# transferia/transferia

Hardware: NVIDIA H100
Metric: ChangeItems/sec on ClickBench-shaped 99-col batches (filter_rows + cast + ClickHouse native block + LZ4 frames) (higher is better)
Workload: dtype u8

## Files before the change

### transferia_b200/csrc/kernels_encode.cuh

```cuda
#pragma once
#include "device_types.cuh"

namespace tfk {

__device__ __forceinline__ uint32_t warp_incl_scan(uint32_t v) {
    const unsigned lane = threadIdx.x & 31;
#pragma unroll
    for (int d = 1; d < 32; d <<= 1) { uint32_t t = __shfl_up_sync(0xffffffffu, v, d); if (lane >= (unsigned)d) v += t; }
    return v;
}
__device__ __forceinline__ uint32_t block_excl_scan(uint32_t v, uint32_t* total, uint32_t* smem33) {
    const unsigned lane = threadIdx.x & 31, warp = threadIdx.x >> 5, nw = (blockDim.x + 31) >> 5;
    uint32_t inc = warp_incl_scan(v);
    if (lane == 31) smem33[warp] = inc;
    __syncthreads();
    if (warp == 0) {
        uint32_t w = lane < nw ? smem33[lane] : 0;
        uint32_t wi = warp_incl_scan(w);
        smem33[lane] = wi - w;
        if (lane == 31) smem33[32] = wi;
    }
    __syncthreads();
    uint32_t res = inc - v + smem33[warp];
    *total = smem33[32];
// ... 363 lines not shown
__global__ void k_layout_columnar(LayoutArgs a, ColRegions* regions);
#ifdef TF_KERNELS_ENCODE
__global__ void __launch_bounds__(256) k_layout_columnar(LayoutArgs a, ColRegions* regions) {
    __shared__ uint64_t s_sz[5][256];
    __shared__ uint64_t s_pos[256];
    __shared__ uint64_t s_run;
    const uint64_t n = a.st->n_kept;
    if (threadIdx.x == 0) s_run = 0;
    for (int base = 0; base < a.ncols; base += 256) {
        const int k = base + threadIdx.x;
        __syncthreads();
        if (k < a.ncols) {
            const DCol& d = a.cols[a.out_cols[k]];
            const bool var = d.out_kind == OK_STR || d.out_kind == OK_MASK || d.out_kind == OK_TOSTR;
            const bool fresh = d.out_kind == OK_MASK || d.out_kind == OK_TOSTR || d.out_kind == OK_TODT;
            const uint64_t heap = (d.out_kind == OK_STR || d.out_kind == OK_TOSTR) ? a.col_bytes[d.str_slot] : (d.out_kind == OK_MASK ? 64 * n : 0);
            s_sz[0][threadIdx.x] = var ? 0 : (uint64_t)d.out_w * n;
            s_sz[1][threadIdx.x] = (d.validity && !fresh) ? (n + 7) / 8 : 0;
            s_sz[2][threadIdx.x] = (d.aux && !fresh) ? (d.type == TF_ANY ? n : 4 * n) : 0;
            s_sz[3][threadIdx.x] = var ? 4 * (n + 1) : 0;
            s_sz[4][threadIdx.x] = heap;
        }
        __syncthreads();
        if (threadIdx.x == 0) {
            uint64_t p = s_run; const int m = a.ncols - base < 256 ? a.ncols - base : 256;
            for (int q = 0; q < m; q++) { s_pos[q] = p; for (int z = 0; z < 5; z++) p += (s_sz[z][q] + 15) & ~15ull; }
            s_run = p;
        }
        __syncthreads();
        if (k < a.ncols) {
            DCol& d = a.cols[a.out_cols[k]];
            uint64_t p = s_pos[threadIdx.x]; ColRegions r;
            auto take = [&](int z) { const uint64_t at = p; p += (s_sz[z][threadIdx.x] + 15) & ~15ull; return at; };
            const uint64_t v = take(0), val = take(1), ax = take(2), of = take(3), hp = take(4);
            const bool var = d.out_kind == OK_STR || d.out_kind == OK_MASK || d.out_kind == OK_TOSTR;
            d.out_off = var ? hp : v; d.null_off = val; d.aux_off = ax; d.offs_off = of;
            r.values = var ? ~0ull : v; r.validity = s_sz[1][threadIdx.x] ? val : ~0ull; r.aux = s_sz[2][threadIdx.x] ? ax : ~0ull;
            r.offsets = var ? of : ~0ull; r.heap = var ? hp : ~0ull; r.heap_len = s_sz[4][threadIdx.x];
            regions[k] = r;
            if (var) ((uint32_t*)(a.raw + of))[n] = (uint32_t)s_sz[4][threadIdx.x];
        }
    }
    __syncthreads();
    if (threadIdx.x == 0) { a.st->raw_total = s_run; a.st->n_frames = 0; a.st->frame_ticket = 0; }
}
#endif

struct EncodeArgs {
    const DCol* cols;
    const int32_t* slots;
    const uint32_t* sel; const DState* st; uint8_t* raw;
    uint32_t* tile_sum; const uint64_t* tile_base; uint32_t ntiles_cap;
    int columnar;
};

#define TF_SLOT_NULLMAP (1 << 30)
#define TF_SLOT_AUX (1 << 29)
#define TF_SLOT_ZEROMAP (1 << 28)
#define TF_FIX_TILE_WORDS 2048
#define CH_MAX_DATE_SEC 4291747200LL

enum StreamKind { SK_COPY = 0, SK_BOOL, SK_DATE, SK_DATETIME, SK_TS64, SK_NULLMAP, SK_AUX32, SK_AUX8, SK_ZERO, SK_TODT_CH, SK_TODT_SEC };

template <int K, int INW> __device__ __forceinline__ uint64_t elem_t(const DCol& c, const uint32_t* sel, uint64_t j, uint64_t n) {
    if (j >= n) return 0;
    const uint64_t r = sel ? sel[j] : j;
    if (K == SK_ZERO) return 0;
    if (K == SK_TODT_CH || K == SK_TODT_SEC) {
        int64_t s = 0;
        if (row_valid(c, r)) s = c.type == TF_INT32 ? (int64_t)((const int32_t*)c.values)[r] : (int64_t)((const uint32_t*)c.values)[r];
        if (K == SK_TODT_SEC) return (uint64_t)s;
        if (s > CH_MAX_DATE_SEC) s = CH_MAX_DATE_SEC;
        if (s < 0) s = 0;
        return (uint64_t)s;
    }
    if (K == SK_AUX8) return (uint64_t)c.aux[r];
    if (K == SK_AUX32) return (uint64_t)((const uint32_t*)c.aux)[r];
    const bool valid = row_valid(c, r);
    if (K == SK_NULLMAP) return valid ? 0 : 1;
    if (!valid) return 0;
    if (K == SK_COPY) {
        if (INW == 1) return c.values[r];
        if (INW == 2) return ((const uint16_t*)c.values)[r];
        if (INW == 4) return ((const uint32_t*)c.values)[r];
        return ((const uint64_t*)c.values)[r];
    }
    if (K == SK_BOOL) return c.values[r] != 0;
    if (K == SK_DATE || K == SK_DATETIME) {
        int64_t s = ((const int64_t*)c.values)[r];
        const uint32_t ns = c.aux ? ((const uint32_t*)c.aux)[r] : 0;
        if (s > CH_MAX_DATE_SEC || (s == CH_MAX_DATE_SEC && ns > 0)) s = CH_MAX_DATE_SEC;
        if (s < 0) s = 0;
        return K == SK_DATE ? (uint64_t)(s / 86400) : (uint64_t)s;
    }
    const int64_t s = ((const int64_t*)c.values)[r];
    const uint32_t ns = c.aux ? ((const uint32_t*)c.aux)[r] : 0;
    return (uint64_t)(s * 1000000LL + (int64_t)(ns / 1000u));
}

template <int K, int INW, int W> __device__ __forceinline__ uint32_t stream_word_t(const DCol& c, const uint32_t* sel, uint64_t q, uint64_t n) {
    if (W == 1) return (uint32_t)elem_t<K, INW>(c, sel, 4 * q, n) | ((uint32_t)elem_t<K, INW>(c, sel, 4 * q + 1, n) << 8) |
                       ((uint32_t)elem_t<K, INW>(c, sel, 4 * q + 2, n) << 16) | ((uint32_t)elem_t<K, INW>(c, sel, 4 * q + 3, n) << 24);
    if (W == 2) return (uint32_t)(elem_t<K, INW>(c, sel, 2 * q, n) & 0xffff) | ((uint32_t)(elem_t<K, INW>(c, sel, 2 * q + 1, n) & 0xffff) << 16);
    if (W == 4) return (uint32_t)elem_t<K, INW>(c, sel, q, n);
    const uint64_t v = elem_t<K, INW>(c, sel, q >> 1, n); return (uint32_t)(v >> ((q & 1) * 32));
}
// ... 105 lines not shown
```

### transferia_b200/csrc/kernels_str.cuh

```cuda
#pragma once
#include "device_types.cuh"
#include "kernels_encode.cuh"
#include "kernels_fmt.cuh"

namespace tfk {

__device__ __forceinline__ uint32_t str_len(const DCol& c, const uint32_t* sel, uint64_t j, uint64_t n, uint64_t& r) {
    if (j >= n) { r = 0; return 0xffffffffu; }
    r = sel ? sel[j] : j;
    if (c.out_kind == OK_TOSTR) { CountSink cs; cs.n = 0; fmt_value(cs, c, r); return cs.n; }
    if (!row_valid(c, r)) return 0;
    return c.offsets[r + 1] - c.offsets[r];
}

#define TF_STR_GROUP 4
__global__ void k_str_sizes(EncodeArgs a);
#ifdef TF_KERNELS_STR
__global__ void __launch_bounds__(TF_STR_THREADS) k_str_sizes(EncodeArgs a) {
    __shared__ uint32_t sm[33];
    const DCol c = a.cols[a.slots[blockIdx.y]];
    const uint64_t n = a.st->n_kept;
    const uint64_t jg = (uint64_t)blockIdx.x * TF_STR_TILE * TF_STR_GROUP;
    if (jg >= n) return;
    uint32_t Ls[TF_STR_GROUP];
#pragma unroll
    for (int g = 0; g < TF_STR_GROUP; g++) { uint64_t r; Ls[g] = str_len(c, a.sel, jg + (uint64_t)g * TF_STR_TILE + threadIdx.x, n, r); }
#pragma unroll
    for (int g = 0; g < TF_STR_GROUP; g++) {
        uint32_t tot; block_excl_scan(Ls[g] != 0xffffffffu ? Ls[g] + (a.columnar ? 0 : varint_len(Ls[g])) : 0u, &tot, sm);
        if (threadIdx.x == 0 && jg + (uint64_t)g * TF_STR_TILE < n) a.tile_sum[(size_t)c.str_slot * a.ntiles_cap + blockIdx.x * TF_STR_GROUP + g] = tot;
        __syncthreads();
    }
}
#endif

__device__ __forceinline__ uint32_t str_find_row(const uint32_t* ex, uint32_t x) {
    uint32_t lo = 0, hi = TF_STR_TILE;
#pragma unroll
    for (int it = 0; it < 8; it++) { const uint32_t mid = (lo + hi) >> 1; if (ex[mid] <= x) lo = mid; else hi = mid; }
    return lo;
}
__global__ void k_encode_str_plain(EncodeArgs a);
#ifdef TF_KERNELS_STR
__global__ void __launch_bounds__(TF_STR_THREADS) k_encode_str_plain(EncodeArgs a) {
    __shared__ uint32_t sm[33];
    __shared__ uint32_t s_ex[TF_STR_GROUP][TF_STR_TILE + 1];
    __shared__ uint32_t s_src[TF_STR_GROUP][TF_STR_TILE];
    __shared__ uint64_t s_tb[TF_STR_GROUP];
    const DCol c = a.cols[a.slots[blockIdx.y]];
    if (c.out_kind == OK_TOSTR) return;
    const uint64_t n = a.st->n_kept;
    const uint64_t jg = (uint64_t)blockIdx.x * TF_STR_TILE * TF_STR_GROUP;
    if (jg >= n) return;
    const uint32_t vlb = a.columnar ? 0u : 1u;
    uint32_t Ls[TF_STR_GROUP]; uint64_t Rs[TF_STR_GROUP]; uint32_t src[TF_STR_GROUP];
#pragma unroll
    for (int g = 0; g < TF_STR_GROUP; g++) Ls[g] = str_len(c, a.sel, jg + (uint64_t)g * TF_STR_TILE + threadIdx.x, n, Rs[g]);
#pragma unroll
    for (int g = 0; g < TF_STR_GROUP; g++) src[g] = (Ls[g] != 0xffffffffu && Ls[g]) ? c.offsets[Rs[g]] : 0u;
#pragma unroll
    for (int g = 0; g < TF_STR_GROUP; g++) {
        const bool have = Ls[g] != 0xffffffffu;
        uint32_t tot; const uint32_t ex = block_excl_scan(have ? Ls[g] + (vlb ? varint_len(Ls[g]) : 0) : 0u, &tot, sm);
        const uint64_t j0 = jg + (uint64_t)g * TF_STR_TILE;
        const uint64_t tb = j0 < n ? a.tile_base[(size_t)c.str_slot * a.ntiles_cap + blockIdx.x * TF_STR_GROUP + g] : 0;
        if (a.columnar && have) ((uint32_t*)(a.raw + c.offs_off))[j0 + threadIdx.x] = (uint32_t)(tb + ex);
        s_ex[g][threadIdx.x] = ex; s_src[g][threadIdx.x] = src[g];
        if (threadIdx.x == 0) { s_ex[g][TF_STR_TILE] = tot; s_tb[g] = tb; }
        __syncthreads();
    }
    const uint32_t hsh = ((uint32_t)(uintptr_t)c.heap & 3);
    const uint32_t* hw = (const uint32_t*)(c.heap - hsh);
#pragma unroll 1
    for (int g = 0; g < TF_STR_GROUP; g++) {
        const uint32_t* ex_ = s_ex[g]; const uint32_t* src_ = s_src[g];
        const uint32_t tot = ex_[TF_STR_TILE];
        if (!tot) continue;
        uint8_t* gdst = a.raw + c.out_off + s_tb[g];
        const uint32_t m = (uint32_t)((uintptr_t)gdst & 3);
        const uint32_t T = (m + tot + 3) >> 2;
        uint8_t* dst0 = gdst - m;
        for (uint32_t t = threadIdx.x; t < T; t += TF_STR_THREADS) {
            const int32_t sb = (int32_t)(4 * t) - (int32_t)m;
            const uint32_t x0 = sb < 0 ? 0u : (uint32_t)sb;
            uint32_t r = str_find_row(ex_, x0);
            uint32_t pe = ex_[r + 1], pl = pe - ex_[r];
            uint32_t plen = pl, vl = 0;
            if (vlb) { vl = pl < 129 ? 1 : (pl < 16386 ? 2 : (pl < 2097155 ? 3 : (pl < 268435460 ? 4 : 5))); plen = pl - vl; }
            const uint32_t k0 = x0 - ex_[r];
            if (sb >= 0 && (uint32_t)sb + 4 <= pe && k0 >= vl) {
                const uint32_t so = src_[r] + (k0 - vl) + hsh; const uint32_t sh = (so & 3) * 8;
                const uint32_t w0 = __ldg(hw + (so >> 2)); uint32_t val = w0;
                if (sh) val = __funnelshift_r(w0, __ldg(hw + (so >> 2) + 1), sh);
                *(uint32_t*)(dst0 + 4 * (size_t)t) = val;
                continue;
            }
            uint32_t val = 0, mask = 0;
#pragma unroll
            for (int b = 0; b < 4; b++) {
                const int32_t xs = sb + b;
                if (xs < 0 || (uint32_t)xs >= tot) continue;
                const uint32_t x = (uint32_t)xs;
                while (x >= pe) { r++; pe = ex_[r + 1]; pl = pe - ex_[r]; if (vlb) { vl = pl < 129 ? 1 : (pl < 16386 ? 2 : (pl < 2097155 ? 3 : (pl < 268435460 ? 4 : 5))); plen = pl - vl; } else plen = pl; }
                const uint32_t k = x - ex_[r];
                uint32_t byte;
                if (k < vl) { const uint32_t v = plen >> (7 * k); byte = (v & 0x7f) | ((v >> 7) ? 0x80u : 0u); }
                else byte = c.heap[src_[r] + (k - vl)];
                val |= byte << (8 * b); mask |= 1u << b;
            }
            uint8_t* dst = dst0 + 4 * (size_t)t;
            if (mask == 15) *(uint32_t*)dst = val;
            else { for (int b = 0; b < 4; b++) if ((mask >> b) & 1) dst[b] = (uint8_t)(val >> (8 * b)); }
        }
    }
}
#endif

__global__ void k_encode_str(EncodeArgs a);
#ifdef TF_KERNELS_STR
__global__ void __launch_bounds__(TF_STR_THREADS) k_encode_str(EncodeArgs a) {
    __shared__ uint32_t sm[33];
    __shared__ __align__(16) uint8_t stage[TF_STR_STAGE + 8];
    const DCol c = a.cols[a.slots[blockIdx.y]];
    if (c.out_kind != OK_TOSTR) return;
    const uint64_t n = a.st->n_kept;
    const uint64_t j0 = (uint64_t)blockIdx.x * TF_STR_TILE;
    if (j0 >= n) return;
    uint64_t R; const uint32_t L = str_len(c, a.sel, j0 + threadIdx.x, n, R);
    if (c.nullable && !a.columnar && L != 0xffffffffu) a.raw[c.null_off + j0 + threadIdx.x] = 0;
    uint32_t tot; const uint32_t ex = block_excl_scan(L != 0xffffffffu ? L + (a.columnar ? 0 : varint_len(L)) : 0u, &tot, sm);
    const uint64_t tb = a.tile_base[(size_t)c.str_slot * a.ntiles_cap + blockIdx.x];
    uint8_t* gdst = a.raw + c.out_off + tb;
    if (a.columnar && L != 0xffffffffu) ((uint32_t*)(a.raw + c.offs_off))[j0 + threadIdx.x] = (uint32_t)(tb + ex);
    const bool staged = tot <= TF_STR_STAGE;
    uint8_t* o = staged ? stage + ex : gdst + ex;
    if (L != 0xffffffffu) {
        if (!a.columnar) {
            uint32_t v = L;
            while (v >= 0x80) { *o++ = (uint8_t)(v | 0x80); v >>= 7; }
            *o++ = (uint8_t)v;
        }
        MemSink ms; ms.p = o; fmt_value(ms, c, R);
    }
    if (!staged) return;
    __syncthreads();
    const uint32_t m = (uint32_t)((uintptr_t)gdst & 3);
    const uint32_t T = (m + tot + 3) >> 2;
    uint8_t* dst0 = gdst - m;
    const uint32_t* sw = (const uint32_t*)stage;
    for (uint32_t t = threadIdx.x; t < T; t += TF_STR_THREADS) {
        const uint32_t wcur = sw[t], wprev = t ? sw[t - 1] : 0;
        const uint32_t val = m ? __funnelshift_r(wprev, wcur, 8 * (4 - m)) : wcur;
        const int32_t sb = (int32_t)(4 * t) - (int32_t)m;
        uint8_t* dst = dst0 + 4 * (size_t)t;
        if (sb >= 0 && (uint32_t)sb + 4 <= tot) *(uint32_t*)dst = val;
        else {
#pragma unroll
            for (int b = 0; b < 4; b++) { const int32_t x = sb + b; if (x >= 0 && (uint32_t)x < tot) dst[b] = (uint8_t)(val >> (8 * b)); }
        }
    }
}
#endif


}
```

### transferia_b200/csrc/tfgpu.cu

```cuda
#include <cuda_runtime.h>
#include <algorithm>
#include <chrono>
#include <cstdio>
#include <cstdlib>
#include <cstring>
#include <memory>
#include <string>
#include <vector>

#include "../../include/tfgpu.h"
#include "../../include/tfgpu_sink.h"
#include "plan.hpp"
#include "device_types.cuh"
#include "launch.hpp"
#include "host_internal.hpp"

using namespace tfk;

namespace {

#define CK(x) do { cudaError_t _e = (x); if (_e != cudaSuccess) throw CudaError{_e, #x}; } while (0)

inline size_t align_up(size_t v, size_t a) { return (v + a - 1) / a * a; }

// ... 357 lines not shown
            if (d.in_w && !d.values) throw tfplan::FatalError(TF_E_FATAL_ARG, "column " + std::to_string(c) + ": values pointer is NULL");
            if (!d.in_w && !d.offsets) throw tfplan::FatalError(TF_E_FATAL_ARG, "column " + std::to_string(c) + ": offsets pointer is NULL");
        }
    }
    const uint16_t* pre_term = nullptr;
    if (!strict.empty() && n) {
        Layout S;
        const size_t o_desc = S.take(strict.size() * sizeof(StrictCol)), o_err = S.take(n), o_term = S.take(2 * n);
        std::vector<size_t> o_val(strict.size());
        for (size_t k = 0; k < strict.size(); k++) o_val[k] = S.take((size_t)in_width(strict[k].dst_tf) * n + 16);
        e->strict_stage.ensure(S.total() + 256);
        uint8_t* B = e->strict_stage.p;
        for (size_t k = 0; k < strict.size(); k++) { strict[k].dst = B + o_val[k]; hc[strict[k].col].values = B + o_val[k]; }
        CK(cudaMemcpyAsync(B + o_desc, strict.data(), strict.size() * sizeof(StrictCol), cudaMemcpyHostToDevice, s));
        if (pre_err) CK(cudaMemcpyAsync(B + o_err, pre_err, n, cudaMemcpyDeviceToDevice, s)); else CK(cudaMemsetAsync(B + o_err, 0, n, s));
        StrictArgs sa{(const StrictCol*)(B + o_desc), (int)strict.size(), n, B + o_err, (uint16_t*)(B + o_term)};
        TF_LAUNCH(e, k_strictify, (uint32_t)((n + 255) / 256), 256, 0, s, sa);
        pre_err = B + o_err; pre_term = (const uint16_t*)(B + o_term);
    }
    CK(cudaMemcpyAsync(e->d_cols, hc.data(), sizeof(DCol) * nc, cudaMemcpyHostToDevice, s));
    CK(cudaMemsetAsync(e->d_state, 0, sizeof(DState), s));
    if (!pl.n2f_cols.empty() && n) {
        const size_t k2 = pl.n2f_cols.size();
        Layout S;
        const size_t o_which = S.take(k2 * 4), o_len = S.take(k2 * n * 4), o_off = S.take(k2 * (n + 1) * 4), o_tot = S.take(k2 * 8 + 8), o_base = S.take(k2 * 8 + 8), o_err = S.take(n);
        e->n2f_stage.ensure(S.total() + 256);
        uint8_t* B = e->n2f_stage.p;
        std::vector<int32_t> which(pl.n2f_cols.begin(), pl.n2f_cols.end());
        CK(cudaMemcpyAsync(B + o_which, which.data(), k2 * 4, cudaMemcpyHostToDevice, s));
        if (pre_err) CK(cudaMemcpyAsync(B + o_err, pre_err, n, cudaMemcpyDeviceToDevice, s)); else CK(cudaMemsetAsync(B + o_err, 0, n, s));
        N2fArgs na{e->d_cols, (const int32_t*)(B + o_which), dev_kinds, n, (uint32_t*)(B + o_len), (const uint32_t*)(B + o_off), nullptr, (const uint64_t*)(B + o_base), B + o_err};
        TF_LAUNCH(e, k_n2f_sizes, dim3((uint32_t)((n + 127) / 128), (uint32_t)k2), 128, 0, s, na);
        const Heaps h = size_heaps(e, (const uint32_t*)(B + o_len), n, (uint32_t)k2, (uint32_t*)(B + o_off), (uint64_t*)(B + o_tot), (uint64_t*)(B + o_base),
                                   e->n2f_heap, "number_to_float: a rewritten column exceeds 4 GiB");
        na.heap = e->n2f_heap.p;
        TF_LAUNCH(e, k_n2f_write, dim3((uint32_t)((n + 127) / 128), (uint32_t)k2), 128, 0, s, na);
        for (size_t k = 0; k < k2; k++) { DCol& d = hc[pl.n2f_cols[k]]; d.offsets = (const uint32_t*)(B + o_off) + k * (n + 1); d.heap = e->n2f_heap.p + h.base[k]; }
        CK(cudaMemcpyAsync(e->d_cols, hc.data(), sizeof(DCol) * nc, cudaMemcpyHostToDevice, s));
        pre_err = B + o_err;
    }
    const bool sink_guard = dev_kinds && !columnar && !dbz;
    const bool has_filter = pd.n_fsteps > 0 || pre_err || sink_guard;
    e->last_wire_fmt = out_fmt;
    const uint32_t nb = (uint32_t)((n + 255) / 256);
    uint32_t* sel = (has_filter && n) ? (uint32_t*)(w + o_sel) : nullptr;
    if (sel) {
        FilterArgs fa{e->d_cols, dev_kinds, n, pd.d_fsteps, pd.n_fsteps, pd.d_expr_off, pd.d_terms, pd.d_blob, keep, errcode, errstep, blockcnt, e->d_state, pre_err, pre_term, sink_guard ? 1 : 0};
        TF_LAUNCH(e, k_filter, nb, 256, 0, s, fa);
        TF_LAUNCH(e, k_scan_blockcnt, 1, 1024, 0, s, blockcnt, blockoff, nb, e->d_state);
        TF_LAUNCH(e, k_compact_sel, nb, 256, 0, s, keep, blockoff, n, sel);
    }
    const uint32_t ntiles = (uint32_t)((n + TF_STR_TILE - 1) / TF_STR_TILE);
    const uint32_t str_gx = std::max(1u, (ntiles + TF_STR_GROUP - 1) / TF_STR_GROUP);
    EncodeArgs ea{e->d_cols, pd.d_str_slots, sel, e->d_state, e->raw.p, tile_sum, tile_base, sz.ntiles_cap, columnar ? 1 : 0};
    if (!has_filter || !n) {
        DState init; std::memset(&init, 0, sizeof init); init.n_kept = n;
        CK(cudaMemcpyAsync(e->d_state, &init, sizeof init, cudaMemcpyHostToDevice, s));
    }
    if (pl.has_sharder && n) {
        e->part_ids.ensure(n * 4 + 256);
        ShardArgs sa{e->d_cols, pd.d_shard_cols, (int)pl.shard_cols.size(), pd.d_mask_keys, sel, e->d_state, pl.shards, (uint32_t*)e->part_ids.p};
        TF_LAUNCH(e, k_shard_ids, nb, 256, 0, s, sa);
    }
    if (json_rows) {
        const uint32_t jt = (uint32_t)((n + TF_JSON_TILE - 1) / TF_JSON_TILE);
        JsonArgs ja{e->d_cols, ser ? (wire_base == TF_WIRE_SER_CSV ? pd.d_scsvcols : pd.d_sjcols) : pd.d_jcols, (int)pl.out_cols.size(), ser ? pd.d_snames : pd.d_jnames, pd.d_mask_keys, sel, e->d_state, e->raw.p,
                    (uint32_t*)e->work_json_sizes(n), tile_sum, tile_base, col_bytes,
                    dbz ? 3 : ser ? (wire_base == TF_WIRE_SER_JSON ? 1 : 2) : 0, (uint32_t)(((out_fmt & TF_WIRE_F_CLOSING_NEWLINE) ? TF_SER_NL : 0) | ((out_fmt & TF_WIRE_F_ANY_AS_STRING) ? TF_SER_AAS : 0)), errcode, errstep, DbzEmitArgs{}};
        if (dbz) { ja.jcols = pd.d_sjcols; e->dbz_keysz.ensure(n * 4 + 256); e->dbz_msgsz.ensure(n * 28 + 256); ja.dz = *dz; ja.dz.key_size = (uint32_t*)e->dbz_keysz.p; ja.dz.msg_size = (uint32_t*)e->dbz_msgsz.p; }
        if (ser && !has_filter && n) { CK(cudaMemsetAsync(errcode, 0, n, s)); CK(cudaMemsetAsync(errstep, 0, 2 * n, s)); }
        if (jt) TF_LAUNCH(e, k_json_sizes, jt, TF_JSON_TILE, 0, s, ja);
        LayoutArgs lj{e->d_cols, 0, pd.d_out_cols, pd.d_str_slots, 1, tile_sum, tile_base, sz.ntiles_cap, pd.d_col_headers, pd.d_col_header_off,
                      e->raw.p, e->d_state, n, 1, e->frame_bytes, col_bytes};
        TF_LAUNCH(e, k_layout_scan, 1, 1024, 0, s, lj);
        uint64_t json_total = 0;
        {
            CK(cudaMemcpyAsync(&json_total, col_bytes, 8, cudaMemcpyDeviceToHost, s)); CK(cudaStreamSynchronize(s));
            e->raw.ensure(json_total + 256); ja.raw = e->raw.p;
        }
        TF_LAUNCH(e, k_json_write, jt ? jt : 1, TF_JSON_TILE, 0, s, ja);
        if (ser && (out_fmt & (TF_WIRE_F_GZIP | TF_WIRE_F_ZLIB))) run_deflate(e, e->raw.p, n ? json_total : 0, (out_fmt & TF_WIRE_F_ZLIB) != 0);
        return ChainOut{errcode, errstep, sel, pl.has_sharder};
    }
    if (pd.n_str && ntiles) TF_LAUNCH(e, k_str_sizes, dim3(str_gx, pd.n_str), TF_STR_THREADS, 0, s, ea);
    LayoutArgs la{e->d_cols, (int)pl.out_cols.size(), pd.d_out_cols, pd.d_str_slots, pd.n_str, tile_sum, tile_base, sz.ntiles_cap, pd.d_col_headers, pd.d_col_header_off,
                  e->raw.p, e->d_state, n, 1, e->frame_bytes, col_bytes};
    if (pd.n_str) TF_LAUNCH(e, k_layout_scan, pd.n_str, 1024, 0, s, la);
    const int32_t* fixed_slots = pd.d_fixed_slots; uint32_t n_fixed = (uint32_t)pd.n_fixed_slots, n_valid = 0;
    if (!columnar) TF_LAUNCH(e, k_layout_finish, 1, 256, 0, s, la);
    else {
        const size_t no = pl.out_cols.size();
        if (e->d_call_cap < no) {
            if (e->d_call_slots) { CK(cudaFree(e->d_call_slots)); CK(cudaFree(e->d_regions)); }
            CK(cudaMalloc(&e->d_call_slots, sizeof(int32_t) * 3 * no)); CK(cudaMalloc(&e->d_regions, sizeof(ColRegions) * no)); e->d_call_cap = no;
        }
        std::vector<int32_t> fixed, valid;
        for (int oc : pl.out_cols) {
            const DCol& d = hc[oc];
            if (d.out_kind == OK_COPY || d.out_kind == OK_TODT) fixed.push_back(oc);
            const bool fresh = d.out_kind == OK_MASK || d.out_kind == OK_TOSTR || d.out_kind == OK_TODT;
            if (!fresh && d.aux) fixed.push_back(oc | TF_SLOT_AUX);
            if (!fresh && d.validity) valid.push_back(oc);
        }
        fixed_slots = e->d_call_slots; n_fixed = (uint32_t)fixed.size(); n_valid = (uint32_t)valid.size();
        fixed.insert(fixed.end(), valid.begin(), valid.end());
        if (!fixed.empty()) CK(cudaMemcpyAsync(e->d_call_slots, fixed.data(), fixed.size() * 4, cudaMemcpyHostToDevice, s));
        TF_LAUNCH(e, k_layout_columnar, 1, 256, 0, s, la, e->d_regions);
    }
    if (n) {
        if (n_fixed) {
            const uint32_t gx = grid_cap(e, (uint32_t)((2 * n + 2 + TF_FIX_TILE_WORDS - 1) / TF_FIX_TILE_WORDS), n_fixed, 6);
            EncodeArgs fa = ea; fa.slots = fixed_slots;
            TF_LAUNCH(e, k_encode_fixed, dim3(gx, n_fixed), 256, 0, s, fa);
        }
        if (n_valid) {
            EncodeArgs va = ea; va.slots = fixed_slots + n_fixed;
            TF_LAUNCH(e, k_pack_validity, dim3((uint32_t)((n / 8 + 256) / 256), n_valid), 256, 0, s, va);
        }
        if (pd.n_str) TF_LAUNCH(e, k_encode_str_plain, dim3(str_gx, pd.n_str), TF_STR_THREADS, 0, s, ea);
        if (pd.n_str && pd.n_tostr) TF_LAUNCH(e, k_encode_str, dim3(ntiles, pd.n_str), TF_STR_THREADS, 0, s, ea);
        if (pd.n_mask_cols) {
            MaskArgs ma{e->d_cols, pd.d_mask_slots, pd.d_mask_keys, sel, e->d_state, e->raw.p, columnar ? 1 : 0};
            TF_LAUNCH(e, k_mask_encode, dim3((uint32_t)((n + 127) / 128), pd.n_mask_cols), 128, 0, s, ma);
        }
    }
    if (lz) {
        Lz4Args za{e->raw.p, e->d_state, e->wire.p, comp_size, wire_off, frame_pfx, e->d_tail, e->frame_bytes, e->lz_phases};
        const size_t smem = lz_smem(e->frame_bytes).total;
        const uint32_t per_sm = (uint32_t)std::max<size_t>(1, std::min<size_t>(LZ_CTAS_PER_SM, (227 * 1024) / (smem + 1024)));
        const uint32_t grid = (uint32_t)std::min<uint64_t>(sz.n_frames_max, (uint64_t)e->sm_count * per_sm);
        join_tail(e);
        CK(cudaMemsetAsync(frame_pfx, 0, sz.n_frames_max * 8, s));
        TF_LAUNCH(e, k_lz4_frames, grid, LZ_THREADS, smem, s, za);
        FrameArgs fa{comp_size, wire_off, e->wire.p, e->d_tail};
        cudaStream_t s3 = e->side_stream;
        CK(cudaEventRecord(e->ev_fork, s)); CK(cudaStreamWaitEvent(s3, e->ev_fork, 0));
        TF_LAUNCH(e, k_frame_seal, (uint32_t)((sz.n_frames_max + 31) / 32), 32, SEAL_SMEM, s3, fa);
// ... 1095 lines not shown
```

Baseline: 1.073 billion.

## Fuse per-column string size kernel across all string slots per tile

k_str_sizes now launches one block per tile group instead of one per (tile, string column). Each block loads the selection indices once and loops over every string slot. It replaces the block exclusive scan, which was only used for its total, with warp __reduce_add_sync sums and a shared-memory reduction. This avoids reading sel once per string column and the many __syncthreads of the per-column scans, but it reduces the grid by a factor of n_str and serializes the columns inside each block, which may lower parallelism.

```diff
diff --git a/transferia_b200/csrc/kernels_encode.cuh b/transferia_b200/csrc/kernels_encode.cuh
--- a/transferia_b200/csrc/kernels_encode.cuh
+++ b/transferia_b200/csrc/kernels_encode.cuh
@@ -439,6 +439,7 @@
     const uint32_t* sel; const DState* st; uint8_t* raw;
     uint32_t* tile_sum; const uint64_t* tile_base; uint32_t ntiles_cap;
     int columnar;
+    int nslots;
 };
 
 #define TF_SLOT_NULLMAP (1 << 30)
diff --git a/transferia_b200/csrc/kernels_str.cuh b/transferia_b200/csrc/kernels_str.cuh
--- a/transferia_b200/csrc/kernels_str.cuh
+++ b/transferia_b200/csrc/kernels_str.cuh
@@ -14,21 +14,50 @@
 }
 
 #define TF_STR_GROUP 4
+#define TF_STR_SLOTS 32
 __global__ void k_str_sizes(EncodeArgs a);
 #ifdef TF_KERNELS_STR
 __global__ void __launch_bounds__(TF_STR_THREADS) k_str_sizes(EncodeArgs a) {
-    __shared__ uint32_t sm[33];
-    const DCol c = a.cols[a.slots[blockIdx.y]];
+    __shared__ uint32_t s_part[TF_STR_SLOTS][TF_STR_GROUP][TF_STR_THREADS / 32];
     const uint64_t n = a.st->n_kept;
     const uint64_t jg = (uint64_t)blockIdx.x * TF_STR_TILE * TF_STR_GROUP;
     if (jg >= n) return;
-    uint32_t Ls[TF_STR_GROUP];
-#pragma unroll
-    for (int g = 0; g < TF_STR_GROUP; g++) { uint64_t r; Ls[g] = str_len(c, a.sel, jg + (uint64_t)g * TF_STR_TILE + threadIdx.x, n, r); }
+    const uint32_t lane = threadIdx.x & 31, warp = threadIdx.x >> 5;
+    uint32_t R[TF_STR_GROUP]; bool in[TF_STR_GROUP];
 #pragma unroll
     for (int g = 0; g < TF_STR_GROUP; g++) {
-        uint32_t tot; block_excl_scan(Ls[g] != 0xffffffffu ? Ls[g] + (a.columnar ? 0 : varint_len(Ls[g])) : 0u, &tot, sm);
-        if (threadIdx.x == 0 && jg + (uint64_t)g * TF_STR_TILE < n) a.tile_sum[(size_t)c.str_slot * a.ntiles_cap + blockIdx.x * TF_STR_GROUP + g] = tot;
+        const uint64_t j = jg + (uint64_t)g * TF_STR_TILE + threadIdx.x;
+        in[g] = j < n; R[g] = in[g] ? (a.sel ? a.sel[j] : (uint32_t)j) : 0u;
+    }
+    for (int s0 = 0; s0 < a.nslots; s0 += TF_STR_SLOTS) {
+        const int ns = min(TF_STR_SLOTS, a.nslots - s0);
+        for (int i = 0; i < ns; i++) {
+            const DCol c = a.cols[a.slots[s0 + i]];
+            uint32_t L[TF_STR_GROUP];
+            if (c.out_kind == OK_TOSTR) {
+#pragma unroll
+                for (int g = 0; g < TF_STR_GROUP; g++) { L[g] = 0; if (in[g]) { CountSink cs; cs.n = 0; fmt_value(cs, c, R[g]); L[g] = cs.n; } }
+            } else {
+                uint32_t o0[TF_STR_GROUP], o1[TF_STR_GROUP]; bool v[TF_STR_GROUP];
+#pragma unroll
+                for (int g = 0; g < TF_STR_GROUP; g++) { o0[g] = __ldg(c.offsets + R[g]); o1[g] = __ldg(c.offsets + R[g] + 1); v[g] = row_valid(c, R[g]); }
+#pragma unroll
+                for (int g = 0; g < TF_STR_GROUP; g++) L[g] = v[g] ? o1[g] - o0[g] : 0u;
+            }
+#pragma unroll
+            for (int g = 0; g < TF_STR_GROUP; g++) {
+                const uint32_t sum = __reduce_add_sync(0xffffffffu, in[g] ? L[g] + (a.columnar ? 0 : varint_len(L[g])) : 0u);
+                if (lane == 0) s_part[i][g][warp] = sum;
+            }
+        }
+        __syncthreads();
+        for (int k = threadIdx.x; k < ns * TF_STR_GROUP; k += TF_STR_THREADS) {
+            const int i = k / TF_STR_GROUP, g = k % TF_STR_GROUP;
+            uint32_t tot = 0;
+#pragma unroll
+            for (int q = 0; q < TF_STR_THREADS / 32; q++) tot += s_part[i][g][q];
+            if (jg + (uint64_t)g * TF_STR_TILE < n) a.tile_sum[(size_t)a.cols[a.slots[s0 + i]].str_slot * a.ntiles_cap + blockIdx.x * TF_STR_GROUP + g] = tot;
+        }
         __syncthreads();
     }
 }
diff --git a/transferia_b200/csrc/tfgpu.cu b/transferia_b200/csrc/tfgpu.cu
--- a/transferia_b200/csrc/tfgpu.cu
+++ b/transferia_b200/csrc/tfgpu.cu
@@ -433,7 +433,7 @@
     }
     const uint32_t ntiles = (uint32_t)((n + TF_STR_TILE - 1) / TF_STR_TILE);
     const uint32_t str_gx = std::max(1u, (ntiles + TF_STR_GROUP - 1) / TF_STR_GROUP);
-    EncodeArgs ea{e->d_cols, pd.d_str_slots, sel, e->d_state, e->raw.p, tile_sum, tile_base, sz.ntiles_cap, columnar ? 1 : 0};
+    EncodeArgs ea{e->d_cols, pd.d_str_slots, sel, e->d_state, e->raw.p, tile_sum, tile_base, sz.ntiles_cap, columnar ? 1 : 0, pd.n_str};
     if (!has_filter || !n) {
         DState init; std::memset(&init, 0, sizeof init); init.n_kept = n;
         CK(cudaMemcpyAsync(e->d_state, &init, sizeof init, cudaMemcpyHostToDevice, s));
@@ -463,7 +463,7 @@
         if (ser && (out_fmt & (TF_WIRE_F_GZIP | TF_WIRE_F_ZLIB))) run_deflate(e, e->raw.p, n ? json_total : 0, (out_fmt & TF_WIRE_F_ZLIB) != 0);
         return ChainOut{errcode, errstep, sel, pl.has_sharder};
     }
-    if (pd.n_str && ntiles) TF_LAUNCH(e, k_str_sizes, dim3(str_gx, pd.n_str), TF_STR_THREADS, 0, s, ea);
+    if (pd.n_str && ntiles) TF_LAUNCH(e, k_str_sizes, str_gx, TF_STR_THREADS, 0, s, ea);
     LayoutArgs la{e->d_cols, (int)pl.out_cols.size(), pd.d_out_cols, pd.d_str_slots, pd.n_str, tile_sum, tile_base, sz.ntiles_cap, pd.d_col_headers, pd.d_col_header_off,
                   e->raw.p, e->d_state, n, 1, e->frame_bytes, col_bytes};
     if (pd.n_str) TF_LAUNCH(e, k_layout_scan, pd.n_str, 1024, 0, s, la);
```

Result: no change. 1.073 billion, median of 6 (+0.0%).

## Batch string-size scans across group and vectorize offset loads in k_str_sizes

Applied to the files above, without the earlier changes.

Rewrites the string sizing kernel so one block-wide scan handles all four tiles of a group at once, with a single barrier, instead of four separate block scans. Offset pairs are read with one 8-byte load when aligned, and validity is read directly. The grid is transposed to columns × row-groups with a grid-stride loop so the row dimension can exceed 65535 blocks. This cuts the synchronisation and load overhead of the sizing pass, but adds register pressure and a specialised path for non-TOSTR columns.

```diff
diff --git a/transferia_b200/csrc/kernels_str.cuh b/transferia_b200/csrc/kernels_str.cuh
--- a/transferia_b200/csrc/kernels_str.cuh
+++ b/transferia_b200/csrc/kernels_str.cuh
@@ -14,21 +14,80 @@
 }
 
 #define TF_STR_GROUP 4
+#define TF_STR_WARPS (TF_STR_THREADS / 32)
+
+__device__ __forceinline__ void str_group_rows(const DCol& c, const uint32_t* sel, uint64_t jg, uint64_t n, uint32_t L[TF_STR_GROUP], uint32_t src[TF_STR_GROUP]) {
+    uint64_t r[TF_STR_GROUP]; bool in[TF_STR_GROUP];
+#pragma unroll
+    for (int g = 0; g < TF_STR_GROUP; g++) {
+        const uint64_t j = jg + (uint64_t)g * TF_STR_TILE + threadIdx.x;
+        in[g] = j < n; r[g] = in[g] ? (sel ? (uint64_t)__ldg(sel + j) : j) : 0;
+    }
+    uint32_t o0[TF_STR_GROUP], o1[TF_STR_GROUP], vb[TF_STR_GROUP];
+#pragma unroll
+    for (int g = 0; g < TF_STR_GROUP; g++) {
+        const uint32_t* p = c.offsets + r[g];
+        o0[g] = o1[g] = 0;
+        if (in[g]) {
+            if (((uintptr_t)p & 7) == 0) { const uint2 v = __ldg((const uint2*)p); o0[g] = v.x; o1[g] = v.y; }
+            else { o0[g] = __ldg(p); o1[g] = __ldg(p + 1); }
+        }
+        vb[g] = (in[g] && c.validity) ? (uint32_t)__ldg(c.validity + (r[g] >> 3)) : 0xffu;
+    }
+#pragma unroll
+    for (int g = 0; g < TF_STR_GROUP; g++) {
+        L[g] = !in[g] ? 0xffffffffu : (((vb[g] >> (r[g] & 7)) & 1) ? o1[g] - o0[g] : 0u);
+        src[g] = o0[g];
+    }
+}
+
+__device__ __forceinline__ void block_excl_scan_group(const uint32_t v[TF_STR_GROUP], uint32_t ex[TF_STR_GROUP], uint32_t tot[TF_STR_GROUP],
+                                                      uint32_t (*sw)[TF_STR_WARPS]) {
+    const unsigned lane = threadIdx.x & 31, warp = threadIdx.x >> 5;
+    uint32_t inc[TF_STR_GROUP];
+#pragma unroll
+    for (int g = 0; g < TF_STR_GROUP; g++) inc[g] = v[g];
+#pragma unroll
+    for (int d = 1; d < 32; d <<= 1) {
+#pragma unroll
+        for (int g = 0; g < TF_STR_GROUP; g++) { const uint32_t t = __shfl_up_sync(0xffffffffu, inc[g], d); if (lane >= (unsigned)d) inc[g] += t; }
+    }
+    if (lane == 31) {
+#pragma unroll
+        for (int g = 0; g < TF_STR_GROUP; g++) sw[g][warp] = inc[g];
+    }
+    __syncthreads();
+#pragma unroll
+    for (int g = 0; g < TF_STR_GROUP; g++) {
+        uint32_t pre = 0, all = 0;
+#pragma unroll
+        for (unsigned w = 0; w < TF_STR_WARPS; w++) { const uint32_t s = sw[g][w]; pre += w < warp ? s : 0u; all += s; }
+        ex[g] = pre + inc[g] - v[g]; tot[g] = all;
+    }
+}
+
 __global__ void k_str_sizes(EncodeArgs a);
 #ifdef TF_KERNELS_STR
 __global__ void __launch_bounds__(TF_STR_THREADS) k_str_sizes(EncodeArgs a) {
-    __shared__ uint32_t sm[33];
-    const DCol c = a.cols[a.slots[blockIdx.y]];
+    __shared__ uint32_t sw[TF_STR_GROUP][TF_STR_WARPS];
     const uint64_t n = a.st->n_kept;
-    const uint64_t jg = (uint64_t)blockIdx.x * TF_STR_TILE * TF_STR_GROUP;
-    if (jg >= n) return;
-    uint32_t Ls[TF_STR_GROUP];
-#pragma unroll
-    for (int g = 0; g < TF_STR_GROUP; g++) { uint64_t r; Ls[g] = str_len(c, a.sel, jg + (uint64_t)g * TF_STR_TILE + threadIdx.x, n, r); }
-#pragma unroll
-    for (int g = 0; g < TF_STR_GROUP; g++) {
-        uint32_t tot; block_excl_scan(Ls[g] != 0xffffffffu ? Ls[g] + (a.columnar ? 0 : varint_len(Ls[g])) : 0u, &tot, sm);
-        if (threadIdx.x == 0 && jg + (uint64_t)g * TF_STR_TILE < n) a.tile_sum[(size_t)c.str_slot * a.ntiles_cap + blockIdx.x * TF_STR_GROUP + g] = tot;
+    if ((uint64_t)blockIdx.y * TF_STR_TILE * TF_STR_GROUP >= n) return;
+    const DCol c = a.cols[a.slots[blockIdx.x]];
+    for (uint32_t grp = blockIdx.y; (uint64_t)grp * TF_STR_TILE * TF_STR_GROUP < n; grp += gridDim.y) {
+        const uint64_t jg = (uint64_t)grp * TF_STR_TILE * TF_STR_GROUP;
+        uint32_t L[TF_STR_GROUP], v[TF_STR_GROUP], ex[TF_STR_GROUP], tot[TF_STR_GROUP];
+        if (c.out_kind == OK_TOSTR) {
+#pragma unroll
+            for (int g = 0; g < TF_STR_GROUP; g++) { uint64_t r; L[g] = str_len(c, a.sel, jg + (uint64_t)g * TF_STR_TILE + threadIdx.x, n, r); }
+        } else {
+            uint32_t src[TF_STR_GROUP]; str_group_rows(c, a.sel, jg, n, L, src);
+        }
+#pragma unroll
+        for (int g = 0; g < TF_STR_GROUP; g++) v[g] = L[g] != 0xffffffffu ? L[g] + (a.columnar ? 0 : varint_len(L[g])) : 0u;
+        block_excl_scan_group(v, ex, tot, sw);
+#pragma unroll
+        for (int g = 0; g < TF_STR_GROUP; g++)
+            if (threadIdx.x == g && jg + (uint64_t)g * TF_STR_TILE < n) a.tile_sum[(size_t)c.str_slot * a.ntiles_cap + grp * TF_STR_GROUP + g] = tot[g];
         __syncthreads();
     }
 }
diff --git a/transferia_b200/csrc/tfgpu.cu b/transferia_b200/csrc/tfgpu.cu
--- a/transferia_b200/csrc/tfgpu.cu
+++ b/transferia_b200/csrc/tfgpu.cu
@@ -433,6 +433,7 @@
     }
     const uint32_t ntiles = (uint32_t)((n + TF_STR_TILE - 1) / TF_STR_TILE);
     const uint32_t str_gx = std::max(1u, (ntiles + TF_STR_GROUP - 1) / TF_STR_GROUP);
+    const dim3 str_grid(pd.n_str, std::min(65535u, str_gx));
     EncodeArgs ea{e->d_cols, pd.d_str_slots, sel, e->d_state, e->raw.p, tile_sum, tile_base, sz.ntiles_cap, columnar ? 1 : 0};
     if (!has_filter || !n) {
         DState init; std::memset(&init, 0, sizeof init); init.n_kept = n;
@@ -463,7 +464,7 @@
         if (ser && (out_fmt & (TF_WIRE_F_GZIP | TF_WIRE_F_ZLIB))) run_deflate(e, e->raw.p, n ? json_total : 0, (out_fmt & TF_WIRE_F_ZLIB) != 0);
         return ChainOut{errcode, errstep, sel, pl.has_sharder};
     }
-    if (pd.n_str && ntiles) TF_LAUNCH(e, k_str_sizes, dim3(str_gx, pd.n_str), TF_STR_THREADS, 0, s, ea);
+    if (pd.n_str && ntiles) TF_LAUNCH(e, k_str_sizes, str_grid, TF_STR_THREADS, 0, s, ea);
     LayoutArgs la{e->d_cols, (int)pl.out_cols.size(), pd.d_out_cols, pd.d_str_slots, pd.n_str, tile_sum, tile_base, sz.ntiles_cap, pd.d_col_headers, pd.d_col_header_off,
                   e->raw.p, e->d_state, n, 1, e->frame_bytes, col_bytes};
     if (pd.n_str) TF_LAUNCH(e, k_layout_scan, pd.n_str, 1024, 0, s, la);
```

New measurement: 1.071 billion before, 1.091 billion after (median of 6 runs). About the same (+1.8%).

## Batch tile scans and flatten plain-string copy into 16-byte chunks with slow-path queue

Applied to the files above, without the earlier changes.

Replaces four sequential block scans with one combined warp-level group scan that uses two barriers, in both the size and encode kernels. The plain string copy now loops over a flattened chunk space spanning all four tiles. Each thread handles a 16-byte chunk and writes it with a single uint4 store when every word is fast-path. Boundary and varint words are compacted into a per-warp shared queue and processed by the whole warp, which cuts divergence. This raises shared memory use and adds a minBlocks launch bound that may limit registers.

```diff
diff --git a/transferia_b200/csrc/kernels_str.cuh b/transferia_b200/csrc/kernels_str.cuh
--- a/transferia_b200/csrc/kernels_str.cuh
+++ b/transferia_b200/csrc/kernels_str.cuh
@@ -14,104 +14,177 @@
 }
 
 #define TF_STR_GROUP 4
+#define TF_STR_WARPS (TF_STR_THREADS / 32)
+static_assert(TF_STR_GROUP <= TF_STR_WARPS, "one warp scans each tile's warp sums");
+
+__device__ __forceinline__ void str_group_scan(uint32_t (&v)[TF_STR_GROUP], uint32_t (*ws)[TF_STR_WARPS + 1]) {
+    const uint32_t lane = threadIdx.x & 31, warp = threadIdx.x >> 5;
+    uint32_t inc[TF_STR_GROUP];
+#pragma unroll
+    for (int g = 0; g < TF_STR_GROUP; g++) inc[g] = warp_incl_scan(v[g]);
+    if (lane == 31) {
+#pragma unroll
+        for (int g = 0; g < TF_STR_GROUP; g++) ws[g][warp] = inc[g];
+    }
+    __syncthreads();
+    if (warp < TF_STR_GROUP) {
+        const uint32_t w = lane < TF_STR_WARPS ? ws[warp][lane] : 0u, wi = warp_incl_scan(w);
+        if (lane < TF_STR_WARPS) ws[warp][lane] = wi - w;
+        if (lane == TF_STR_WARPS - 1) ws[warp][TF_STR_WARPS] = wi;
+    }
+    __syncthreads();
+#pragma unroll
+    for (int g = 0; g < TF_STR_GROUP; g++) v[g] = inc[g] - v[g] + ws[g][warp];
+}
+
 __global__ void k_str_sizes(EncodeArgs a);
 #ifdef TF_KERNELS_STR
 __global__ void __launch_bounds__(TF_STR_THREADS) k_str_sizes(EncodeArgs a) {
-    __shared__ uint32_t sm[33];
-    const DCol c = a.cols[a.slots[blockIdx.y]];
+    __shared__ uint32_t s_ws[TF_STR_GROUP][TF_STR_WARPS + 1];
     const uint64_t n = a.st->n_kept;
+    const int32_t slot = a.slots[blockIdx.y];
     const uint64_t jg = (uint64_t)blockIdx.x * TF_STR_TILE * TF_STR_GROUP;
     if (jg >= n) return;
+    const DCol c = a.cols[slot];
     uint32_t Ls[TF_STR_GROUP];
 #pragma unroll
     for (int g = 0; g < TF_STR_GROUP; g++) { uint64_t r; Ls[g] = str_len(c, a.sel, jg + (uint64_t)g * TF_STR_TILE + threadIdx.x, n, r); }
 #pragma unroll
-    for (int g = 0; g < TF_STR_GROUP; g++) {
-        uint32_t tot; block_excl_scan(Ls[g] != 0xffffffffu ? Ls[g] + (a.columnar ? 0 : varint_len(Ls[g])) : 0u, &tot, sm);
-        if (threadIdx.x == 0 && jg + (uint64_t)g * TF_STR_TILE < n) a.tile_sum[(size_t)c.str_slot * a.ntiles_cap + blockIdx.x * TF_STR_GROUP + g] = tot;
-        __syncthreads();
-    }
+    for (int g = 0; g < TF_STR_GROUP; g++) Ls[g] = Ls[g] != 0xffffffffu ? Ls[g] + (a.columnar ? 0 : varint_len(Ls[g])) : 0u;
+    str_group_scan(Ls, s_ws);
+    if (threadIdx.x < TF_STR_GROUP && jg + (uint64_t)threadIdx.x * TF_STR_TILE < n)
+        a.tile_sum[(size_t)c.str_slot * a.ntiles_cap + blockIdx.x * TF_STR_GROUP + threadIdx.x] = s_ws[threadIdx.x][TF_STR_WARPS];
 }
 #endif
 
+#define TF_STR_CHUNK_WORDS 4
 __device__ __forceinline__ uint32_t str_find_row(const uint32_t* ex, uint32_t x) {
     uint32_t lo = 0, hi = TF_STR_TILE;
 #pragma unroll
     for (int it = 0; it < 8; it++) { const uint32_t mid = (lo + hi) >> 1; if (ex[mid] <= x) lo = mid; else hi = mid; }
     return lo;
 }
+__device__ __forceinline__ uint32_t str_piece_vl(uint32_t pl) {
+    return pl < 129 ? 1 : (pl < 16386 ? 2 : (pl < 2097155 ? 3 : (pl < 268435460 ? 4 : 5)));
+}
+__device__ __forceinline__ void str_word_bytes(const uint32_t* ex_, const uint32_t* src_, const uint8_t* heap, uint32_t vlb, int32_t sb,
+                                               uint32_t r, uint8_t* dst) {
+    const uint32_t tot = ex_[TF_STR_TILE];
+    uint32_t ps = ex_[r], pe = ex_[r + 1], val = 0, mask = 0;
+#pragma unroll
+    for (int b = 0; b < 4; b++) {
+        const int32_t xs = sb + b;
+        if (xs < 0 || (uint32_t)xs >= tot) continue;
+        const uint32_t x = (uint32_t)xs;
+        while (x >= pe) { r++; ps = pe; pe = ex_[r + 1]; }
+        const uint32_t pl = pe - ps, vl = vlb ? str_piece_vl(pl) : 0, k = x - ps;
+        uint32_t byte;
+        if (k < vl) { const uint32_t v = (pl - vl) >> (7 * k); byte = (v & 0x7f) | ((v >> 7) ? 0x80u : 0u); }
+        else byte = heap[src_[r] + (k - vl)];
+        val |= byte << (8 * b); mask |= 1u << b;
+    }
+    if (mask == 15) *(uint32_t*)dst = val;
+    else { for (int b = 0; b < 4; b++) if ((mask >> b) & 1) dst[b] = (uint8_t)(val >> (8 * b)); }
+}
 __global__ void k_encode_str_plain(EncodeArgs a);
 #ifdef TF_KERNELS_STR
-__global__ void __launch_bounds__(TF_STR_THREADS) k_encode_str_plain(EncodeArgs a) {
-    __shared__ uint32_t sm[33];
+__global__ void __launch_bounds__(TF_STR_THREADS, 2048 / TF_STR_THREADS) k_encode_str_plain(EncodeArgs a) {
+    constexpr uint32_t CB = 4 * TF_STR_CHUNK_WORDS;
+    static_assert(TF_STR_CHUNK_WORDS == 4, "a whole chunk is one uint4 store");
+    __shared__ uint32_t s_ws[TF_STR_GROUP][TF_STR_WARPS + 1];
     __shared__ uint32_t s_ex[TF_STR_GROUP][TF_STR_TILE + 1];
     __shared__ uint32_t s_src[TF_STR_GROUP][TF_STR_TILE];
     __shared__ uint64_t s_tb[TF_STR_GROUP];
-    const DCol c = a.cols[a.slots[blockIdx.y]];
-    if (c.out_kind == OK_TOSTR) return;
+    __shared__ uint32_t s_cp[TF_STR_GROUP + 1];
+    __shared__ uint2 s_q[TF_STR_WARPS][32 * TF_STR_CHUNK_WORDS];
     const uint64_t n = a.st->n_kept;
+    const int32_t slot = a.slots[blockIdx.y];
     const uint64_t jg = (uint64_t)blockIdx.x * TF_STR_TILE * TF_STR_GROUP;
     if (jg >= n) return;
+    const DCol c = a.cols[slot];
+    if (c.out_kind == OK_TOSTR) return;
     const uint32_t vlb = a.columnar ? 0u : 1u;
+    if (threadIdx.x < TF_STR_GROUP) {
+        const uint64_t j0 = jg + (uint64_t)threadIdx.x * TF_STR_TILE;
+        s_tb[threadIdx.x] = j0 < n ? a.tile_base[(size_t)c.str_slot * a.ntiles_cap + blockIdx.x * TF_STR_GROUP + threadIdx.x] : 0;
+    }
     uint32_t Ls[TF_STR_GROUP]; uint64_t Rs[TF_STR_GROUP]; uint32_t src[TF_STR_GROUP];
 #pragma unroll
     for (int g = 0; g < TF_STR_GROUP; g++) Ls[g] = str_len(c, a.sel, jg + (uint64_t)g * TF_STR_TILE + threadIdx.x, n, Rs[g]);
 #pragma unroll
     for (int g = 0; g < TF_STR_GROUP; g++) src[g] = (Ls[g] != 0xffffffffu && Ls[g]) ? c.offsets[Rs[g]] : 0u;
 #pragma unroll
+    for (int g = 0; g < TF_STR_GROUP; g++) Ls[g] = Ls[g] != 0xffffffffu ? Ls[g] + (vlb ? varint_len(Ls[g]) : 0) : 0u;
+    str_group_scan(Ls, s_ws);
+    uint32_t cp = 0;
+#pragma unroll
     for (int g = 0; g < TF_STR_GROUP; g++) {
-        const bool have = Ls[g] != 0xffffffffu;
-        uint32_t tot; const uint32_t ex = block_excl_scan(have ? Ls[g] + (vlb ? varint_len(Ls[g]) : 0) : 0u, &tot, sm);
-        const uint64_t j0 = jg + (uint64_t)g * TF_STR_TILE;
-        const uint64_t tb = j0 < n ? a.tile_base[(size_t)c.str_slot * a.ntiles_cap + blockIdx.x * TF_STR_GROUP + g] : 0;
-        if (a.columnar && have) ((uint32_t*)(a.raw + c.offs_off))[j0 + threadIdx.x] = (uint32_t)(tb + ex);
+        const uint32_t ex = Ls[g], tot = s_ws[g][TF_STR_WARPS];
+        const uint64_t tb = s_tb[g];
+        const uint64_t j = jg + (uint64_t)g * TF_STR_TILE + threadIdx.x;
+        if (a.columnar && j < n) ((uint32_t*)(a.raw + c.offs_off))[j] = (uint32_t)(tb + ex);
         s_ex[g][threadIdx.x] = ex; s_src[g][threadIdx.x] = src[g];
-        if (threadIdx.x == 0) { s_ex[g][TF_STR_TILE] = tot; s_tb[g] = tb; }
-        __syncthreads();
-    }
+        if (tot) cp += ((uint32_t)((uintptr_t)(a.raw + c.out_off + tb) & (CB - 1)) + tot + CB - 1) / CB;
+        if (threadIdx.x == 0) { s_ex[g][TF_STR_TILE] = tot; s_cp[g + 1] = cp; }
+    }
+    if (threadIdx.x == 0) s_cp[0] = 0;
+    __syncthreads();
     const uint32_t hsh = ((uint32_t)(uintptr_t)c.heap & 3);
     const uint32_t* hw = (const uint32_t*)(c.heap - hsh);
-#pragma unroll 1
-    for (int g = 0; g < TF_STR_GROUP; g++) {
-        const uint32_t* ex_ = s_ex[g]; const uint32_t* src_ = s_src[g];
-        const uint32_t tot = ex_[TF_STR_TILE];
-        if (!tot) continue;
-        uint8_t* gdst = a.raw + c.out_off + s_tb[g];
-        const uint32_t m = (uint32_t)((uintptr_t)gdst & 3);
-        const uint32_t T = (m + tot + 3) >> 2;
-        uint8_t* dst0 = gdst - m;
-        for (uint32_t t = threadIdx.x; t < T; t += TF_STR_THREADS) {
-            const int32_t sb = (int32_t)(4 * t) - (int32_t)m;
-            const uint32_t x0 = sb < 0 ? 0u : (uint32_t)sb;
-            uint32_t r = str_find_row(ex_, x0);
-            uint32_t pe = ex_[r + 1], pl = pe - ex_[r];
-            uint32_t plen = pl, vl = 0;
-            if (vlb) { vl = pl < 129 ? 1 : (pl < 16386 ? 2 : (pl < 2097155 ? 3 : (pl < 268435460 ? 4 : 5))); plen = pl - vl; }
-            const uint32_t k0 = x0 - ex_[r];
-            if (sb >= 0 && (uint32_t)sb + 4 <= pe && k0 >= vl) {
-                const uint32_t so = src_[r] + (k0 - vl) + hsh; const uint32_t sh = (so & 3) * 8;
-                const uint32_t w0 = __ldg(hw + (so >> 2)); uint32_t val = w0;
-                if (sh) val = __funnelshift_r(w0, __ldg(hw + (so >> 2) + 1), sh);
-                *(uint32_t*)(dst0 + 4 * (size_t)t) = val;
-                continue;
+    const uint32_t lane = threadIdx.x & 31, warp = threadIdx.x >> 5;
+    for (uint32_t f0 = threadIdx.x & ~31u; f0 < cp; f0 += TF_STR_THREADS) {
+        const uint32_t f = f0 + lane;
+        uint32_t slow = 0, rs = 0, g = 0, ci = 0;
+        if (f < cp) {
+            while (f >= s_cp[g + 1]) g++;
+            const uint32_t* ex_ = s_ex[g]; const uint32_t* src_ = s_src[g];
+            const uint32_t tot = ex_[TF_STR_TILE];
+            uint8_t* gdst = a.raw + c.out_off + s_tb[g];
+            const uint32_t m = (uint32_t)((uintptr_t)gdst & (CB - 1));
+            ci = f - s_cp[g];
+            uint8_t* dst = gdst - m + (size_t)CB * ci;
+            const int32_t sb0 = (int32_t)(CB * ci) - (int32_t)m;
+            uint32_t r = str_find_row(ex_, sb0 < 0 ? 0u : (uint32_t)sb0);
+            uint32_t ps = ex_[r], pe = ex_[r + 1];
+            uint32_t lo[TF_STR_CHUNK_WORDS], hi[TF_STR_CHUNK_WORDS], sh = 0, full = 0;
+#pragma unroll
+            for (int w = 0; w < TF_STR_CHUNK_WORDS; w++) {
+                lo[w] = 0; hi[w] = 0;
+                const int32_t sb = sb0 + 4 * w;
+                const uint32_t x0 = sb < 0 ? 0u : (uint32_t)sb;
+                if (sb <= -4 || x0 >= tot) continue;
+                while (x0 >= pe) { r++; ps = pe; pe = ex_[r + 1]; }
+                const uint32_t vl = vlb ? str_piece_vl(pe - ps) : 0, k0 = x0 - ps;
+                if (sb >= 0 && (uint32_t)sb + 4 <= pe && k0 >= vl) {
+                    const uint32_t so = src_[r] + (k0 - vl) + hsh;
+                    lo[w] = __ldg(hw + (so >> 2));
+                    if (so & 3) hi[w] = __ldg(hw + (so >> 2) + 1);
+                    sh |= (so & 3) << (8 * w); full |= 1u << w;
+                } else { slow |= 1u << w; rs |= r << (8 * w); }
             }
-            uint32_t val = 0, mask = 0;
-#pragma unroll
-            for (int b = 0; b < 4; b++) {
-                const int32_t xs = sb + b;
-                if (xs < 0 || (uint32_t)xs >= tot) continue;
-                const uint32_t x = (uint32_t)xs;
-                while (x >= pe) { r++; pe = ex_[r + 1]; pl = pe - ex_[r]; if (vlb) { vl = pl < 129 ? 1 : (pl < 16386 ? 2 : (pl < 2097155 ? 3 : (pl < 268435460 ? 4 : 5))); plen = pl - vl; } else plen = pl; }
-                const uint32_t k = x - ex_[r];
-                uint32_t byte;
-                if (k < vl) { const uint32_t v = plen >> (7 * k); byte = (v & 0x7f) | ((v >> 7) ? 0x80u : 0u); }
-                else byte = c.heap[src_[r] + (k - vl)];
-                val |= byte << (8 * b); mask |= 1u << b;
+#pragma unroll
+            for (int w = 0; w < TF_STR_CHUNK_WORDS; w++) lo[w] = __funnelshift_r(lo[w], hi[w], 8 * ((sh >> (8 * w)) & 3));
+            if (full == (1u << TF_STR_CHUNK_WORDS) - 1) *(uint4*)dst = make_uint4(lo[0], lo[1], lo[2], lo[3]);
+            else {
+#pragma unroll
+                for (int w = 0; w < TF_STR_CHUNK_WORDS; w++) if ((full >> w) & 1) ((uint32_t*)dst)[w] = lo[w];
             }
-            uint8_t* dst = dst0 + 4 * (size_t)t;
-            if (mask == 15) *(uint32_t*)dst = val;
-            else { for (int b = 0; b < 4; b++) if ((mask >> b) & 1) dst[b] = (uint8_t)(val >> (8 * b)); }
-        }
+        }
+        const uint32_t cnt = __popc(slow), qe = warp_incl_scan(cnt), qn = __shfl_sync(0xffffffffu, qe, 31);
+        uint2* q = s_q[warp];
+        for (uint32_t i = qe - cnt; slow; slow &= slow - 1, i++) {
+            const uint32_t w = __ffs(slow) - 1;
+            q[i] = make_uint2(TF_STR_CHUNK_WORDS * ci + w, g | (((rs >> (8 * w)) & 255) << 8));
+        }
+        __syncwarp();
+        for (uint32_t e = lane; e < qn; e += 32) {
+            const uint2 it = q[e];
+            const uint32_t qg = it.y & 255;
+            uint8_t* gdst = a.raw + c.out_off + s_tb[qg];
+            const uint32_t m = (uint32_t)((uintptr_t)gdst & (CB - 1));
+            str_word_bytes(s_ex[qg], s_src[qg], c.heap, vlb, (int32_t)(4 * it.x) - (int32_t)m, it.y >> 8, gdst - m + 4 * (size_t)it.x);
+        }
+        __syncwarp();
     }
 }
 #endif
```

Result: faster. 1.073 billion before, 1.164 billion after, median of 6 (+8.5%).
